# Layr-Labs/rust-kzg-bn254

Measured on AMD Instinct MI355X. Metric: G1-MSM (scalar,point) pairs/s = 2^20 x KZG coeff-form commitments/s, 2^20-point SRS, higher is better.
Workload: dtype int32x9 (29-bit limbs, 64-bit accumulate); 1 GPU; G1 MSM 2^20 scalars (KZG::commit_coeff_form), scalars resident in HBM; step k commits buffer k mod 8 (8 distinct resident scalar sets, 256 MiB); pipeline_depth=2, steps_per_launch=1

## Files before the change

rust-kzg-bn254_amd/csrc/msm_kernels.h:

```cpp
#pragma once
#include <hip/hip_runtime.h>
#include "curve_pair.h"
#include "curve_quad.h"
#include "naf.h"
#include "msm_limits.h"

namespace kzg {

__device__ __forceinline__ void latency_bound_kernel() {
#if !defined(KZG_NO_SETPRIO)
    __builtin_amdgcn_s_setprio(3);
#endif
}

constexpr uint32_t DIGIT_NONE = 0xFFFFFFFFu;

__global__ void __launch_bounds__(256)
k_msm_digits(const uint4* __restrict__ scalars, uint32_t n_total, uint32_t n, int c, int W, uint32_t* __restrict__ digits,
             uint32_t* __restrict__ count = nullptr ) {
    latency_bound_kernel();
    uint32_t j = blockIdx.x * blockDim.x + threadIdx.x;
    if (j >= n_total) return;
    const uint32_t msm = j / n, i = j - msm * n;
    uint4 lo = scalars[2 * (size_t)j], hi = scalars[2 * (size_t)j + 1];
    uint32_t w32[8] = {lo.x, lo.y, lo.z, lo.w, hi.x, hi.y, hi.z, hi.w};
    uint32_t k[8];
    fe_wire_to_canonical_words<FrParams>(k, w32);
    const uint32_t mask = (1u << c) - 1u, half = 1u << (c - 1);
    uint32_t carry = 0;
    for (int w = 0; w < W; ++w) {
        uint32_t raw = (k[0] & mask) + carry;
#pragma unroll
        for (int j = 0; j < 7; ++j) k[j] = (k[j] >> c) | (k[j + 1] << (32 - c));
        k[7] >>= c;
        uint32_t neg = raw > half;
        uint32_t mag = neg ? (1u << c) - raw : raw;
        carry = neg;
        uint32_t v = DIGIT_NONE;
        if (mag != 0) {
            v = (mag - 1) | (neg << 31);
            if (count) atomicAdd(&count[mag - 1], 1u);
        }
        digits[((size_t)msm * W + w) * n + i] = v;
    }
}


template <int T>
__device__ __forceinline__ uint32_t block_excl_scan(uint32_t v, uint32_t* total, uint32_t* lds ) {
    const int t = threadIdx.x;
    lds[t] = v;
    __syncthreads();
    for (int d = 1; d < T; d <<= 1) {
        uint32_t x = (t >= d) ? lds[t - d] : 0u;
        __syncthreads();
        lds[t] += x;
        __syncthreads();
    }
    uint32_t incl = lds[t];
    *total = lds[T - 1];
    __syncthreads();
    return incl - v;
}
__device__ __forceinline__ uint4 scan1_load(const uint32_t* __restrict__ count, uint32_t g, uint32_t hi) {
    if (g + 4 <= hi) return *reinterpret_cast<const uint4*>(count + g);
    uint4 v = make_uint4(0, 0, 0, 0);
    if (g < hi) v.x = count[g];
    if (g + 1 < hi) v.y = count[g + 1];
    if (g + 2 < hi) v.z = count[g + 2];
    return v;
}
template <bool LEAN>
__global__ void __launch_bounds__(SCAN1_THREADS)
k_scan_counts_1wg(uint32_t* __restrict__ count, uint32_t G, uint32_t* __restrict__ offs , uint32_t* __restrict__ cursor ) {
    latency_bound_kernel();
    __shared__ uint32_t wave_total[SCAN1_THREADS / 64];
    const uint32_t t = threadIdx.x, w = t >> 6, lane = t & 63;
    const uint32_t per_wave = (((G + SCAN1_THREADS / 64 - 1) / (SCAN1_THREADS / 64)) + 255u) & ~255u;
    const uint32_t lo = min(G, w * per_wave), hi = min(G, lo + per_wave);
    uint32_t s = 0;
    for (uint32_t g0 = lo; g0 < hi; g0 += 1024) {
        const uint32_t g = g0 + lane * 4;
        const uint4 a = scan1_load(count, g, hi), b = scan1_load(count, g + 256, hi), c = scan1_load(count, g + 512, hi), d = scan1_load(count, g + 768, hi);
        s += a.x + a.y + a.z + a.w + b.x + b.y + b.z + b.w + c.x + c.y + c.z + c.w + d.x + d.y + d.z + d.w;
    }
    for (int d = 32; d >= 1; d >>= 1) s += __shfl_xor(s, d, 64);
    if (lane == 0) wave_total[w] = s;
    __syncthreads();
    uint32_t run = 0, total = 0;
    for (uint32_t q = 0; q < SCAN1_THREADS / 64; ++q) { const uint32_t x = wave_total[q]; if (q < w) run += x; total += x; }
    for (uint32_t g0 = lo; g0 < hi; g0 += 1024) {
        uint4 v[4];
#pragma unroll
        for (int k = 0; k < 4; ++k) v[k] = scan1_load(count, g0 + k * 256 + lane * 4, hi);
#pragma unroll
        for (int k = 0; k < 4; ++k) {
            const uint32_t g = g0 + k * 256 + lane * 4;
            const uint32_t sum4 = v[k].x + v[k].y + v[k].z + v[k].w;
            uint32_t incl = sum4;
            for (int d = 1; d < 64; d <<= 1) { const uint32_t x = __shfl_up(incl, d, 64); if ((int)lane >= d) incl += x; }
            uint4 o;
            o.x = run + incl - sum4; o.y = o.x + v[k].x; o.z = o.y + v[k].y; o.w = o.z + v[k].z;
            if (g + 4 <= hi) {
                *reinterpret_cast<uint4*>(offs + g) = o;
                if (LEAN) { *reinterpret_cast<uint4*>(cursor + g) = o; *reinterpret_cast<uint4*>(count + g) = make_uint4(0, 0, 0, 0); }
            } else {
                if (g < hi) { offs[g] = o.x; if (LEAN) { cursor[g] = o.x; count[g] = 0; } }
                if (g + 1 < hi) { offs[g + 1] = o.y; if (LEAN) { cursor[g + 1] = o.y; count[g + 1] = 0; } }
                if (g + 2 < hi) { offs[g + 2] = o.z; if (LEAN) { cursor[g + 2] = o.z; count[g + 2] = 0; } }
            }
            run += __shfl(incl, 63, 64);
        }
    }
    if (t == 0) offs[G] = total;
}
__global__ void __launch_bounds__(SCAN_THREADS)
k_scan_block_sums(const uint32_t* __restrict__ count, uint32_t G, uint32_t* __restrict__ block_sums) {
    __shared__ uint32_t lds[SCAN_THREADS];
    size_t base = (size_t)blockIdx.x * SCAN_TILE + (size_t)threadIdx.x * SCAN_ITEMS;
    uint32_t s = 0;
#pragma unroll
    for (int j = 0; j < SCAN_ITEMS; ++j) if (base + j < G) s += count[base + j];
    uint32_t total;
    block_excl_scan<SCAN_THREADS>(s, &total, lds);
    if (threadIdx.x == 0) block_sums[blockIdx.x] = total;
}
__global__ void __launch_bounds__(SCAN_THREADS)
k_scan_top(uint32_t* __restrict__ block_sums, uint32_t nb) {
    __shared__ uint32_t lds[SCAN_THREADS];
    size_t base = (size_t)threadIdx.x * SCAN_ITEMS;
    uint32_t v[SCAN_ITEMS], s = 0;
#pragma unroll
    for (int j = 0; j < SCAN_ITEMS; ++j) { v[j] = (base + j < nb) ? block_sums[base + j] : 0u; s += v[j]; }
    uint32_t total;
    uint32_t pre = block_excl_scan<SCAN_THREADS>(s, &total, lds);
#pragma unroll
    for (int j = 0; j < SCAN_ITEMS; ++j) { if (base + j < nb) block_sums[base + j] = pre; pre += v[j]; }
}
__global__ void __launch_bounds__(SCAN_THREADS)
k_scan_final(const uint32_t* __restrict__ count, uint32_t G, const uint32_t* __restrict__ block_sums,
             uint32_t* __restrict__ offs ) {
    __shared__ uint32_t lds[SCAN_THREADS];
    size_t base = (size_t)blockIdx.x * SCAN_TILE + (size_t)threadIdx.x * SCAN_ITEMS;
    uint32_t v[SCAN_ITEMS], s = 0;
#pragma unroll
    for (int j = 0; j < SCAN_ITEMS; ++j) { v[j] = (base + j < G) ? count[base + j] : 0u; s += v[j]; }
    uint32_t total;
    uint32_t pre = block_excl_scan<SCAN_THREADS>(s, &total, lds) + block_sums[blockIdx.x];
#pragma unroll
    for (int j = 0; j < SCAN_ITEMS; ++j) { if (base + j < G) offs[base + j] = pre; pre += v[j]; }
    if (blockIdx.x == gridDim.x - 1 && threadIdx.x == SCAN_THREADS - 1) offs[G] = pre;
}

__global__ void __launch_bounds__(256)
k_sort_hist(const uint32_t* __restrict__ digits, uint32_t set_len, uint32_t tile_len, uint32_t tiles_per_set, uint32_t B,
            uint32_t* __restrict__ count, uint32_t* __restrict__ blockbase) {
    latency_bound_kernel();
    extern __shared__ uint32_t lds_u32[];
    const uint32_t set = blockIdx.x / tiles_per_set, tile = blockIdx.x % tiles_per_set;
    const uint32_t lo = tile * tile_len;
    const uint32_t hi = (set_len - lo < tile_len) ? set_len : lo + tile_len;
    for (uint32_t b = threadIdx.x; b < B; b += blockDim.x) lds_u32[b] = 0;
    __syncthreads();
    const uint32_t* d = digits + (size_t)set * set_len;
    for (uint32_t e = lo + threadIdx.x; e < hi; e += blockDim.x) {
        uint32_t v = d[e];
        if (v != DIGIT_NONE) atomicAdd(&lds_u32[v & 0x7FFFFFFFu], 1u);
    }
    __syncthreads();
    for (uint32_t b = threadIdx.x; b < B; b += blockDim.x) {
        uint32_t h = lds_u32[b];
        uint32_t base = h ? atomicAdd(&count[(size_t)set * B + b], h) : 0u;
        blockbase[(size_t)blockIdx.x * B + b] = base;
    }
}
__global__ void __launch_bounds__(256)
k_sort_scatter(const uint32_t* __restrict__ digits, uint32_t n, uint32_t set_len, uint32_t tile_len, uint32_t tiles_per_set, uint32_t B,
               const uint32_t* __restrict__ offs, const uint32_t* __restrict__ blockbase, uint32_t table_stride,
               uint32_t windows_per_msm, uint32_t* __restrict__ sorted) {
    latency_bound_kernel();
    extern __shared__ uint32_t lds_u32[];
    const uint32_t set = blockIdx.x / tiles_per_set, tile = blockIdx.x % tiles_per_set;
    const uint32_t base_idx = table_stride ? 0u : (set / windows_per_msm) * n;
    const uint32_t lo = tile * tile_len;
    const uint32_t hi = (set_len - lo < tile_len) ? set_len : lo + tile_len;
    for (uint32_t b = threadIdx.x; b < B; b += blockDim.x)
        lds_u32[b] = offs[(size_t)set * B + b] + blockbase[(size_t)blockIdx.x * B + b];
    __syncthreads();
    const uint32_t* d = digits + (size_t)set * set_len;
    for (uint32_t e = lo + threadIdx.x; e < hi; e += blockDim.x) {
        uint32_t v = d[e];
        if (v == DIGIT_NONE) continue;
        uint32_t pos = atomicAdd(&lds_u32[v & 0x7FFFFFFFu], 1u);
        uint32_t idx;
        if (table_stride) { uint32_t w = e / n; idx = w * table_stride + (e - w * n); }
        else idx = base_idx + e;
        sorted[pos] = idx | (v & 0x80000000u);
    }
}

__global__ void __launch_bounds__(256)
k_sort_small_hist(const uint32_t* __restrict__ digits, uint32_t n_entries, uint32_t set_len, uint32_t B, uint32_t* __restrict__ count) {
    latency_bound_kernel();
    const uint32_t e = blockIdx.x * blockDim.x + threadIdx.x;
    if (e >= n_entries) return;
    const uint32_t v = digits[e];
    if (v != DIGIT_NONE) atomicAdd(&count[(size_t)(e / set_len) * B + (v & 0x7FFFFFFFu)], 1u);
}
__global__ void __launch_bounds__(256)
k_sort_small_scatter(const uint32_t* __restrict__ digits, uint32_t n_entries, uint32_t n, uint32_t set_len, uint32_t B,
                     const uint32_t* __restrict__ offs, uint32_t* __restrict__ cursor , uint32_t table_stride,
                     uint32_t windows_per_msm, uint32_t* __restrict__ sorted, int cursor_is_offs = 0) {
    latency_bound_kernel();
    const uint32_t e = blockIdx.x * blockDim.x + threadIdx.x;
    if (e >= n_entries) return;
    const uint32_t v = digits[e];
    if (v == DIGIT_NONE) return;
    const uint32_t set = e / set_len, es = e - set * set_len;
    const size_t gb = (size_t)set * B + (v & 0x7FFFFFFFu);
    const uint32_t pos = (cursor_is_offs ? 0u : offs[gb]) + atomicAdd(&cursor[gb], 1u);
    uint32_t idx;
    if (table_stride) { const uint32_t w = es / n; idx = w * table_stride + (es - w * n); }
    else idx = (set / windows_per_msm) * n + es;
    sorted[pos] = idx | (v & 0x80000000u);
}


template <bool SCATTER>
__global__ void __launch_bounds__(256)
k_sort2_scalars(const uint4* __restrict__ scalars, uint32_t n, int c, int W, uint32_t tile_s, uint32_t Hb, uint32_t* __restrict__ ccount,
                uint32_t* __restrict__ blockbase1, const uint32_t* __restrict__ cstart, uint32_t table_stride, uint32_t* __restrict__ tmp1) {
    latency_bound_kernel();
    extern __shared__ uint32_t lds_u32[];
    const uint32_t lo = blockIdx.x * tile_s;
    const uint32_t hi = (n - lo < tile_s) ? n : lo + tile_s;
    for (uint32_t b = threadIdx.x; b < Hb; b += blockDim.x) lds_u32[b] = SCATTER ? cstart[b] + blockbase1[(size_t)blockIdx.x * Hb + b] : 0u;
    __syncthreads();
    const uint32_t mask = (1u << c) - 1u, half = 1u << (c - 1);
    for (uint32_t i = lo + threadIdx.x; i < hi; i += blockDim.x) {
        const uint4 s_lo = scalars[2 * (size_t)i], s_hi = scalars[2 * (size_t)i + 1];
        uint32_t w32[8] = {s_lo.x, s_lo.y, s_lo.z, s_lo.w, s_hi.x, s_hi.y, s_hi.z, s_hi.w};
        uint32_t k[8];
        fe_wire_to_canonical_words<FrParams>(k, w32);
        uint32_t carry = 0, idx = i;
        for (int w = 0; w < W; ++w, idx += table_stride) {
            const uint32_t raw = (k[0] & mask) + carry;
#pragma unroll
            for (int j = 0; j < 7; ++j) k[j] = (k[j] >> c) | (k[j + 1] << (32 - c));
            k[7] >>= c;
            const uint32_t neg = raw > half;
            const uint32_t mag = neg ? (1u << c) - raw : raw;
            carry = neg;
            if (mag == 0) continue;
            const uint32_t key = mag - 1;
            if (SCATTER) {
                const uint32_t pos = atomicAdd(&lds_u32[key >> SORT2_LO_BITS], 1u);
                tmp1[pos] = (neg << 31) | ((key & (SORT2_LO - 1)) << SORT2_IDX_BITS) | idx;
            } else {
                atomicAdd(&lds_u32[key >> SORT2_LO_BITS], 1u);
            }
        }
    }
    if (SCATTER) return;
    __syncthreads();
    for (uint32_t b = threadIdx.x; b < Hb; b += blockDim.x) {
        const uint32_t h = lds_u32[b];
        blockbase1[(size_t)blockIdx.x * Hb + b] = h ? atomicAdd(&ccount[b], h) : 0u;
    }
}
struct PolyPtrs { const uint4* p[MSM_BATCH_PTRS]; };
template <int ND>
__global__ void __launch_bounds__(256)
k_naf_digits(const uint4* __restrict__ scalars, uint32_t n, int c, uint32_t tile_s, uint32_t Hb, uint32_t* __restrict__ ccount,
             uint32_t* __restrict__ blockbase1, uint4* __restrict__ digs, uint32_t poly_len, PolyPtrs ptrs) {
    latency_bound_kernel();
    extern __shared__ uint32_t lds_u32[];
    uint32_t* hist = lds_u32;
    uint32_t* col = hist + Hb + threadIdx.x;
    uint32_t* stage = hist + Hb + 11 * 256;
    const uint32_t t = threadIdx.x;
    const uint32_t lo = blockIdx.x * tile_s;
    const uint32_t hi = (n - lo < tile_s) ? n : lo + tile_s;
    for (uint32_t b = t; b < Hb; b += 256) hist[b] = 0u;
    col[8 * 256] = 0; col[9 * 256] = 0; col[10 * 256] = 0;
    for (uint32_t base = lo; base < hi; base += 256) {
        __syncthreads();
#pragma unroll
        for (int m = 0; m < ND; ++m) stage[m * 256 + t] = NAF_NO_DIGIT;
        const uint32_t i = base + t;
        if (i < hi) {
            const uint4* sp = scalars + 2 * (size_t)i;
            if (poly_len && ptrs.p[0]) {
                const uint32_t pk = i / poly_len;
                const uint4* base = ptrs.p[0];
#pragma unroll
                for (int q = 1; q < MSM_BATCH_PTRS; ++q) base = pk == (uint32_t)q ? ptrs.p[q] : base;
                sp = base + 2 * (size_t)(i - pk * poly_len);
            }
            const uint4 s_lo = sp[0], s_hi = sp[1];
            uint32_t w32[8] = {s_lo.x, s_lo.y, s_lo.z, s_lo.w, s_hi.x, s_hi.y, s_hi.z, s_hi.w};
            uint32_t k[8];
            fe_wire_to_canonical_words<FrParams>(k, w32);
#pragma unroll
            for (int j = 0; j < 8; ++j) col[j * 256] = k[j];
            uint32_t m = 0;
            const uint32_t group = poly_len ? (i / poly_len) << (c - 1) : 0u;
            naf_for_digits_lds(col, 256, c + 1, [&](uint32_t pos, uint32_t key, uint32_t neg) {
                const uint32_t g = group | (c - 1 > 6 ? naf_bucket(key, c - 1) : key);
                atomicAdd(&hist[g >> SORT2_LO_BITS], 1u);
                if (m < (uint32_t)ND) stage[m * 256 + t] = (neg << 31) | (pos << 16) | g;
                ++m;
            });
        }
        __syncthreads();
#pragma unroll
        for (int r = 0; r < ND / 4; ++r) {
            const uint32_t idx = t + 256 * r, sc = idx / (ND / 4), q = idx % (ND / 4);
            if (base + sc < hi)
                digs[(size_t)(base + sc) * (ND / 4) + q] = make_uint4(stage[(4 * q) * 256 + sc], stage[(4 * q + 1) * 256 + sc],
                                                                    stage[(4 * q + 2) * 256 + sc], stage[(4 * q + 3) * 256 + sc]);
        }
    }
    __syncthreads();
    for (uint32_t b = t; b < Hb; b += 256) {
        const uint32_t h = hist[b];
        blockbase1[(size_t)blockIdx.x * Hb + b] = h ? atomicAdd(&ccount[b], h) : 0u;
    }
}
static_assert(SORT2_MAX_BINS <= 512 && SORT2_LO_BITS == 7, "LDS entry layout of k_sort2_scatter1_lds");
template <class F>
__device__ __forceinline__ void sort2_for_digits(uint32_t k[8], int c, int W, F&& f) {
    const uint32_t mask = (1u << c) - 1u, half = 1u << (c - 1);
    uint32_t carry = 0;
    for (int w = 0; w < W; ++w) {
        const uint32_t raw = (k[0] & mask) + carry;
#pragma unroll
        for (int j = 0; j < 7; ++j) k[j] = (k[j] >> c) | (k[j + 1] << (32 - c));
        k[7] >>= c;
        const uint32_t neg = raw > half;
        const uint32_t mag = neg ? (1u << c) - raw : raw;
        carry = neg;
        if (mag != 0) f((uint32_t)w, mag - 1, neg);
    }
}
template <bool NAF = false, int ND = NAF_DIGITS>
__global__ void __launch_bounds__(SORT2_P1_THREADS)
k_sort2_scatter1_lds(const uint4* __restrict__ scalars, uint32_t n, int c, int W, uint32_t tile_s, uint32_t Hb, const uint32_t* __restrict__ blockbase1,
                     const uint32_t* __restrict__ cstart, uint32_t table_stride, uint32_t* __restrict__ tmp1, uint8_t* __restrict__ tmpk = nullptr,
                     uint32_t poly_len = 0) {
    latency_bound_kernel();
    extern __shared__ uint32_t lds_u32[];
    uint32_t* gpos = lds_u32;
    uint32_t* hist = gpos + Hb;
    uint32_t* lstart = hist + Hb;
    uint32_t* buf = lstart + Hb;
    uint16_t* bufk = reinterpret_cast<uint16_t*>(buf + (size_t)SORT2_P1_THREADS * W);
    const uint32_t t = threadIdx.x, lane = t & 63;
    const uint32_t lo = blockIdx.x * tile_s;
    const uint32_t hi = (n - lo < tile_s) ? n : lo + tile_s;
    for (uint32_t b = t; b < Hb; b += SORT2_P1_THREADS) gpos[b] = cstart[b] + blockbase1[(size_t)blockIdx.x * Hb + b];
    const uint32_t per_lane = (Hb + 63) / 64;
    for (uint32_t base = lo; base < hi; base += SORT2_P1_THREADS) {
        __syncthreads();
        for (uint32_t b = t; b < Hb; b += SORT2_P1_THREADS) hist[b] = 0;
        __syncthreads();
        const uint32_t i = base + t;
        const bool have = i < hi;
        uint32_t kk[8] = {0, 0, 0, 0, 0, 0, 0, 0};
        uint32_t dg[NAF ? ND : 1];
        if (NAF) {
#pragma unroll
            for (int m = 0; m < (NAF ? ND : 1); ++m) dg[m] = NAF_NO_DIGIT;
            if (have) {
                const uint4* src = reinterpret_cast<const uint4*>(scalars) + (size_t)i * (ND / 4);
#pragma unroll
                for (int q = 0; q < (NAF ? ND / 4 : 0); ++q) {
                    const uint4 v = src[q];
                    dg[4 * q] = v.x; dg[4 * q + 1] = v.y; dg[4 * q + 2] = v.z; dg[4 * q + 3] = v.w;
                }
                bool live = true;
#pragma unroll
                for (int m = 0; m < (NAF ? ND : 0); ++m) {
                    live = live && dg[m] != NAF_NO_DIGIT;
                    if (!live) dg[m] = NAF_NO_DIGIT;
                    else atomicAdd(&hist[(dg[m] & 0xFFFFu) >> SORT2_LO_BITS], 1u);
                }
            }
        } else
        if (have) {
            const uint4 s_lo = scalars[2 * (size_t)i], s_hi = scalars[2 * (size_t)i + 1];
            const uint32_t w32[8] = {s_lo.x, s_lo.y, s_lo.z, s_lo.w, s_hi.x, s_hi.y, s_hi.z, s_hi.w};
            fe_wire_to_canonical_words<FrParams>(kk, w32);
            uint32_t k[8];
#pragma unroll
            for (int j = 0; j < 8; ++j) k[j] = kk[j];
            sort2_for_digits(k, c, W, [&](uint32_t, uint32_t key, uint32_t) { atomicAdd(&hist[key >> SORT2_LO_BITS], 1u); });
        }
        __syncthreads();
        if (t < 64) {
            uint32_t sum = 0;
            for (uint32_t q = 0; q < per_lane; ++q) { const uint32_t b = lane * per_lane + q; if (b < Hb) sum += hist[b]; }
            uint32_t incl = sum;
            for (int d = 1; d < 64; d <<= 1) { const uint32_t x = __shfl_up(incl, d, 64); if ((int)lane >= d) incl += x; }
            uint32_t run = incl - sum;
            for (uint32_t q = 0; q < per_lane; ++q) {
                const uint32_t b = lane * per_lane + q;
                if (b < Hb) { lstart[b] = run; run += hist[b]; }
            }
        }
        __syncthreads();
        const uint32_t cn = lstart[Hb - 1] + hist[Hb - 1];
        __syncthreads();
        for (uint32_t b = t; b < Hb; b += SORT2_P1_THREADS) hist[b] = 0;
        __syncthreads();
        if (have) {
            if (NAF) {
#pragma unroll
                for (int m = 0; m < (NAF ? ND : 0); ++m) {
                    if (dg[m] == NAF_NO_DIGIT) continue;
                    const uint32_t key = dg[m] & 0xFFFFu;
                    const uint32_t bin = key >> SORT2_LO_BITS;
                    const uint32_t slot = lstart[bin] + atomicAdd(&hist[bin], 1u);
                    buf[slot] = (dg[m] & 0x80000000u) | (((dg[m] >> 16) & 255u) << 9) | t;
                    bufk[slot] = (uint16_t)key;
                }
            } else {
                sort2_for_digits(kk, c, W, [&](uint32_t w, uint32_t key, uint32_t neg) {
                    const uint32_t bin = key >> SORT2_LO_BITS;
                    const uint32_t slot = lstart[bin] + atomicAdd(&hist[bin], 1u);
                    buf[slot] = (bin << 22) | ((key & (SORT2_LO - 1)) << 15) | (neg << 14) | (w << 9) | t;
                });
            }
        }
        __syncthreads();
        if (NAF) {
            for (uint32_t q = t; q < cn; q += SORT2_P1_THREADS) {
                const uint32_t x = buf[q], key = bufk[q], bin = key >> SORT2_LO_BITS;
                const uint32_t sidx = base + (x & 511u);
                const uint32_t idx = ((x >> 9) & 255u) * table_stride + (poly_len ? sidx % poly_len : sidx);
                const uint32_t dst = gpos[bin] + (q - lstart[bin]);
                tmp1[dst] = (x & 0x80000000u) | idx;
                tmpk[dst] = (uint8_t)(key & (SORT2_LO - 1));
            }
        } else
        for (uint32_t q = t; q < cn; q += SORT2_P1_THREADS) {
            const uint32_t x = buf[q], bin = x >> 22;
            const uint32_t idx = ((x >> 9) & 31u) * table_stride + base + (x & 511u);
            tmp1[gpos[bin] + (q - lstart[bin])] = ((x >> 14) & 1u) << 31 | ((x >> 15) & (SORT2_LO - 1)) << SORT2_IDX_BITS | idx;
        }
        __syncthreads();
        for (uint32_t b = t; b < Hb; b += SORT2_P1_THREADS) gpos[b] += hist[b];
    }
}
__global__ void __launch_bounds__(512)
k_sort2_scan(const uint32_t* __restrict__ ccount, uint32_t Hb, uint32_t* __restrict__ cstart, uint32_t* __restrict__ tstart,
             uint32_t* __restrict__ tile_bin, uint32_t* __restrict__ count, uint32_t* __restrict__ cap_out) {
    latency_bound_kernel();
    __shared__ uint32_t a[512], b[512];
    __shared__ uint32_t total;
    const uint32_t t = threadIdx.x;
    uint32_t c = t < Hb ? ccount[t] : 0u;
    if (t == 0) total = 0;
    __syncthreads();
    if (c) atomicAdd(&total, c);
    __syncthreads();
    const uint32_t cap_dyn = total / Hb + total / Hb / 4 + 2048u;
    const uint32_t cap = cap_dyn < SORT2_BIN_CAP ? cap_dyn : SORT2_BIN_CAP;
    if (t == 0) *cap_out = cap;
    uint32_t k = c > cap ? (c + SORT2_CHUNK - 1) / SORT2_CHUNK : 0u;
    a[t] = c; b[t] = k;
    __syncthreads();
    for (uint32_t d = 1; d < 512; d <<= 1) {
        uint32_t x = t >= d ? a[t - d] : 0u, y = t >= d ? b[t - d] : 0u;
        __syncthreads();
        a[t] += x; b[t] += y;
        __syncthreads();
    }
    if (t < Hb) {
        cstart[t] = a[t] - c; tstart[t] = b[t] - k;
        for (uint32_t q = b[t] - k; q < b[t]; ++q) tile_bin[q] = t;
        if (k) for (uint32_t q = 0; q < SORT2_LO; ++q) count[(size_t)t * SORT2_LO + q] = 0u;
    }
    if (t == Hb - 1) { cstart[Hb] = a[t]; tstart[Hb] = b[t]; }
}
template <bool NAF>
__device__ __forceinline__ uint32_t sort2_low_key(const uint32_t* __restrict__ tmp1, const uint8_t* __restrict__ tmpk, uint32_t e) {
    return NAF ? (uint32_t)tmpk[e] : (tmp1[e] >> SORT2_IDX_BITS) & (SORT2_LO - 1);
}
template <bool NAF = false>
__global__ void __launch_bounds__(256)
k_sort2_hist2(const uint32_t* __restrict__ tmp1, const uint32_t* __restrict__ cstart, const uint32_t* __restrict__ tstart,
              const uint32_t* __restrict__ tile_bin, uint32_t Hb, uint32_t* __restrict__ count, uint32_t* __restrict__ blockbase2,
              const uint8_t* __restrict__ tmpk = nullptr) {
    latency_bound_kernel();
    __shared__ uint32_t hist[SORT2_LO];
    const uint32_t tile = blockIdx.x;
    if (tile >= tstart[Hb]) return;
    const uint32_t h = tile_bin[tile];
    const uint32_t lo = cstart[h] + (tile - tstart[h]) * SORT2_CHUNK;
    const uint32_t hi = (cstart[h + 1] - lo < SORT2_CHUNK) ? cstart[h + 1] : lo + SORT2_CHUNK;
    if (threadIdx.x < SORT2_LO) hist[threadIdx.x] = 0;
    __syncthreads();
    for (uint32_t e = lo + threadIdx.x; e < hi; e += blockDim.x) atomicAdd(&hist[sort2_low_key<NAF>(tmp1, tmpk, e)], 1u);
    __syncthreads();
    if (threadIdx.x < SORT2_LO) {
        uint32_t c = hist[threadIdx.x];
        blockbase2[(size_t)tile * SORT2_LO + threadIdx.x] = c ? atomicAdd(&count[(size_t)h * SORT2_LO + threadIdx.x], c) : 0u;
    }
}
template <bool NAF = false>
__global__ void __launch_bounds__(256)
k_sort2_scatter2(const uint32_t* __restrict__ tmp1, const uint32_t* __restrict__ cstart, const uint32_t* __restrict__ tstart,
                 const uint32_t* __restrict__ tile_bin, uint32_t Hb, const uint32_t* __restrict__ offs,
                 const uint32_t* __restrict__ blockbase2, uint32_t* __restrict__ sorted, const uint8_t* __restrict__ tmpk = nullptr) {
    latency_bound_kernel();
    __shared__ uint32_t cur[SORT2_LO];
    const uint32_t tile = blockIdx.x;
    if (tile >= tstart[Hb]) return;
    const uint32_t h = tile_bin[tile];
    const uint32_t lo = cstart[h] + (tile - tstart[h]) * SORT2_CHUNK;
    const uint32_t hi = (cstart[h + 1] - lo < SORT2_CHUNK) ? cstart[h + 1] : lo + SORT2_CHUNK;
    if (threadIdx.x < SORT2_LO)
        cur[threadIdx.x] = offs[(size_t)h * SORT2_LO + threadIdx.x] + blockbase2[(size_t)tile * SORT2_LO + threadIdx.x];
    __syncthreads();
    for (uint32_t e = lo + threadIdx.x; e < hi; e += blockDim.x) {
        uint32_t v = tmp1[e];
        uint32_t pos = atomicAdd(&cur[sort2_low_key<NAF>(tmp1, tmpk, e)], 1u);
        sorted[pos] = NAF ? v : v & (0x80000000u | SORT2_IDX_MASK);
    }
}

template <bool NAF = false>
__global__ void __launch_bounds__(SORT2_BIN_THREADS)
k_sort2_bin(const uint32_t* __restrict__ tmp1, const uint32_t* __restrict__ cstart, uint32_t Hb, const uint32_t* __restrict__ count,
            uint32_t* __restrict__ offs, uint32_t* __restrict__ sorted, const uint32_t* __restrict__ cap_ptr, const uint8_t* __restrict__ tmpk = nullptr) {
    latency_bound_kernel();
    __shared__ uint32_t hist[SORT2_LO], gpos[SORT2_LO], lstart[SORT2_LO], buf[SORT2_BIN_CHUNK];
    __shared__ uint8_t bufk[NAF ? SORT2_BIN_CHUNK : 4];
    const uint32_t h = blockIdx.x, t = threadIdx.x;
    const uint32_t lo = cstart[h], hi = cstart[h + 1];
    const bool large = hi - lo > *cap_ptr;
    if (t < SORT2_LO) hist[t] = large ? count[(size_t)h * SORT2_LO + t] : 0u;
    __syncthreads();
    if (!large) {
        uint32_t e = lo + t;
        for (; e + 3 * SORT2_BIN_THREADS < hi; e += 4 * SORT2_BIN_THREADS) {
            const uint32_t k0 = sort2_low_key<NAF>(tmp1, tmpk, e), k1 = sort2_low_key<NAF>(tmp1, tmpk, e + SORT2_BIN_THREADS),
                           k2 = sort2_low_key<NAF>(tmp1, tmpk, e + 2 * SORT2_BIN_THREADS), k3 = sort2_low_key<NAF>(tmp1, tmpk, e + 3 * SORT2_BIN_THREADS);
            atomicAdd(&hist[k0], 1u);
            atomicAdd(&hist[k1], 1u);
            atomicAdd(&hist[k2], 1u);
            atomicAdd(&hist[k3], 1u);
        }
        for (; e < hi; e += SORT2_BIN_THREADS) atomicAdd(&hist[sort2_low_key<NAF>(tmp1, tmpk, e)], 1u);
        __syncthreads();
    }
    static_assert(SORT2_LO == 128, "two counters per lane of one wave");
    if (t < 64) {
        const uint32_t c0 = hist[2 * t], c1 = hist[2 * t + 1];
        uint32_t incl = c0 + c1;
        for (int d = 1; d < 64; d <<= 1) { const uint32_t x = __shfl_up(incl, d, 64); if ((int)t >= d) incl += x; }
        const uint32_t start = lo + incl - (c0 + c1);
        gpos[2 * t] = start; gpos[2 * t + 1] = start + c0;
        offs[(size_t)h * SORT2_LO + 2 * t] = start;
        offs[(size_t)h * SORT2_LO + 2 * t + 1] = start + c0;
    }
    if (h == Hb - 1 && t == 0) offs[(size_t)Hb * SORT2_LO] = cstart[Hb];
    if (large) return;
    for (uint32_t base = lo; base < hi; base += SORT2_BIN_CHUNK) {
        const uint32_t cn = hi - base < SORT2_BIN_CHUNK ? hi - base : SORT2_BIN_CHUNK;
        __syncthreads();
        if (t < SORT2_LO) hist[t] = 0;
        __syncthreads();
        uint32_t v[SORT2_BIN_PER], r[SORT2_BIN_PER], kq[SORT2_BIN_PER];
#pragma unroll
        for (int j = 0; j < SORT2_BIN_PER; ++j) {
            const uint32_t i = j * SORT2_BIN_THREADS + t;
            v[j] = i < cn ? tmp1[base + i] : 0u;
            kq[j] = NAF ? (i < cn ? (uint32_t)tmpk[base + i] : 0u) : (v[j] >> SORT2_IDX_BITS) & (SORT2_LO - 1);
        }
#pragma unroll
        for (int j = 0; j < SORT2_BIN_PER; ++j)
            if (j * SORT2_BIN_THREADS + t < cn) r[j] = atomicAdd(&hist[kq[j]], 1u);
        __syncthreads();
        if (t < 64) {
            const uint32_t c0 = hist[2 * t], c1 = hist[2 * t + 1];
            uint32_t incl = c0 + c1;
            for (int d = 1; d < 64; d <<= 1) { const uint32_t x = __shfl_up(incl, d, 64); if ((int)t >= d) incl += x; }
            lstart[2 * t] = incl - (c0 + c1); lstart[2 * t + 1] = incl - c1;
        }
        __syncthreads();
#pragma unroll
        for (int j = 0; j < SORT2_BIN_PER; ++j)
            if (j * SORT2_BIN_THREADS + t < cn) {
                const uint32_t slot = lstart[kq[j]] + r[j];
                buf[slot] = v[j];
                if (NAF) bufk[slot] = (uint8_t)kq[j];
            }
        __syncthreads();
        for (uint32_t i = t; i < cn; i += SORT2_BIN_THREADS) {
            const uint32_t x = buf[i], k = NAF ? (uint32_t)bufk[i] : (x >> SORT2_IDX_BITS) & (SORT2_LO - 1);
            sorted[gpos[k] + (i - lstart[k])] = NAF ? x : x & (0x80000000u | SORT2_IDX_MASK);
        }
        __syncthreads();
        if (t < SORT2_LO) gpos[t] += hist[t];
    }
}

#ifndef KZG_RUN_SERIAL
#define KZG_RUN_SERIAL 8
#endif
constexpr uint32_t RUN_SERIAL = KZG_RUN_SERIAL;
constexpr uint32_t NP_SERIAL = 10;

__device__ __forceinline__ uint32_t acc_seg_len(uint32_t E, uint32_t nl) { return (E + nl - 1) / nl; }

#ifdef KZG_ACC_NOGATHER
#define KZG_ACC_IDX(v) ((v) & 0xFFu)
#else
#define KZG_ACC_IDX(v) ((v) & 0x7FFFFFFFu)
#endif
__device__ __forceinline__ size_t acc_point_index(uint32_t ix, uint32_t idx_log, uint32_t stride_adj) {
    return (size_t)ix + (size_t)(ix >> idx_log) * stride_adj;
}
#ifndef KZG_ACC_WAVES
#define KZG_ACC_WAVES 3
#endif
#ifdef KZG_TEST_HOOKS
__device__ unsigned long long g_acc_replays;
#endif
__device__ __noinline__ Xyzz acc_replay(const uint4* __restrict__ points, const uint32_t* __restrict__ sorted, uint32_t lo, uint32_t hi, uint32_t idx_log, uint32_t stride_adj) {
    Xyzz r;
    xyzz_set_inf(r);
#pragma unroll 1
    for (uint32_t e = lo; e < hi; ++e) {
        const uint32_t v = sorted[e];
        Affine p;
        if (!affine_load(p, points + 4 * acc_point_index(KZG_ACC_IDX(v), idx_log, stride_adj))) continue;
        xyzz_madd<true>(r, p, v >> 31);
    }
#ifdef KZG_TEST_HOOKS
    atomicAdd(&g_acc_replays, 1ull);
#endif
    return r;
}
template <bool IDENTITY_BASES>
__global__ void __launch_bounds__(256) __attribute__((amdgpu_waves_per_eu(KZG_ACC_WAVES, KZG_ACC_WAVES)))
k_msm_accumulate(const uint4* __restrict__ points, const uint32_t* __restrict__ sorted, const uint32_t* __restrict__ offs, uint32_t G,
                 int32_t* __restrict__ head, size_t head_stride, int32_t* __restrict__ cont, size_t cont_stride,
                 uint32_t idx_log, uint32_t stride_adj) {
    const uint32_t nl = gridDim.x * blockDim.x;
    const uint32_t t = blockIdx.x * blockDim.x + threadIdx.x;
    const uint32_t lane = threadIdx.x & 63;
#ifdef KZG_ACC_STAMPS
    unsigned long long* stamps = reinterpret_cast<unsigned long long*>(cont + cont_stride * 36) + 8 * (size_t)(t >> 6);
    const unsigned long long stamp0 = __builtin_amdgcn_s_memrealtime();
    unsigned long long flush_ticks = 0, flush_events = 0, stamp_loop = 0;
#endif
    const uint32_t E = offs[G];
    const uint32_t L = acc_seg_len(E, nl);
    const unsigned long long b64 = (unsigned long long)t * L;
    const uint32_t begin = b64 < E ? (uint32_t)b64 : E;
    const uint32_t end = (b64 + L < E) ? (uint32_t)(b64 + L) : E;
    const bool active = begin < end;
    uint32_t g = 0, next = 0, g0 = 0xFFFFFFFFu;
    bool is_cont = false, long_run = false;
    if (active) {
        uint32_t lo = 0, hi = G;
#ifdef KZG_ACC_BINARY_SEARCH
        while (hi - lo > 1) {
            const uint32_t mid = (lo + hi) >> 1;
            if (offs[mid] <= begin) lo = mid; else hi = mid;
        }
#else
        while (hi - lo > 1) {
            const uint32_t s = (hi - lo + 15) >> 4;
            uint32_t cnt = 0;
#pragma unroll
            for (uint32_t j = 1; j < 16; ++j) {
                const uint32_t p = lo + j * s;
                const uint32_t v = p < hi ? offs[p] : 0xFFFFFFFFu;
                cnt += v <= begin ? 1u : 0u;
            }
            const uint32_t nlo = lo + cnt * s, nhi = lo + (cnt + 1) * s;
            if (cnt < 15 && nhi < hi) hi = nhi;
            lo = nlo;
        }
#endif
        g = lo;
        const uint32_t o0 = offs[g];
        next = offs[g + 1];
        is_cont = o0 < begin;
        if (is_cont) { long_run = ((next - 1) / L - o0 / L) > RUN_SERIAL; g0 = g; }
    }
    __shared__ int32_t park[4 * NL * 256];
    const uint32_t tl = threadIdx.x;
    bool parked = false, parked_cont = false;
    uint32_t park_g = 0;
    bool cont_in_regs = false;
    Xyzz acc;
    xyzz_set_inf(acc);
    uint32_t next2 = 0;
    if (active) next2 = offs[g + 2 <= G ? g + 2 : G];
    auto flush = [&](bool more) {
        if (__builtin_expect(!acc.inf && fe_is_zero_mod(acc.zz), 0)) {
            const uint32_t o0 = offs[g], o1 = offs[g + 1];
            acc = acc_replay(points, sorted, o0 > begin ? o0 : begin, o1 < end ? o1 : end, idx_log, stride_adj);
        }
        KZG_REQUIRE(!acc.inf || (fe_is_literal_zero(acc.x) && fe_is_literal_zero(acc.y) && fe_is_literal_zero(acc.zz) && fe_is_literal_zero(acc.zzz)),
                    KZG_SITE_IS_ZERO_MOD, "k_msm_accumulate: inf without zero limbs", acc.zz);
        const bool as_cont = is_cont && g == g0;
        if (more && !parked) {
            const Fq* c4[4] = {&acc.x, &acc.y, &acc.zz, &acc.zzz};
#pragma unroll
            for (int q = 0; q < 4; ++q)
#pragma unroll
                for (int j = 0; j < NL; ++j) park[(q * NL + j) * 256 + tl] = c4[q]->l[j];
            parked = true; parked_cont = as_cont; park_g = g;
        } else if (!as_cont) {
            xyzz_store_zeroed(head, head_stride, g, acc);
        } else if (!long_run || more) {
            xyzz_store_zeroed(cont, cont_stride, t, acc);
        } else {
            cont_in_regs = true;
        }
    };
#ifdef KZG_ACC_STAMPS
    stamp_loop = __builtin_amdgcn_s_memrealtime();
#endif
    if (active) {
        const uint32_t last = end - 1;
        uint32_t v = sorted[begin];
        uint32_t v1 = sorted[begin + 1 < end ? begin + 1 : last];
        typedef uint32_t u32x4 __attribute__((ext_vector_type(4)));
        const u32x4* const pts = reinterpret_cast<const u32x4*>(points);
        const u32x4* src = pts + 4 * acc_point_index(KZG_ACC_IDX(v), idx_log, stride_adj);
        u32x4 q0 = src[0], q1 = src[1], q2 = src[2], q3 = src[3];
        for (uint32_t e = begin; e < end; ++e) {
#ifdef KZG_ACC_STAMPS
            const bool any_cross = __any(e == next);
            unsigned long long f0 = 0;
            if (any_cross) f0 = __builtin_amdgcn_s_memrealtime();
#endif
            if (__builtin_expect(e == next, 0)) {
                flush(true);
                xyzz_set_inf(acc);
                ++g; next = next2;
                while (next == e) { ++g; next = offs[g + 1]; }
                next2 = offs[g + 2 <= G ? g + 2 : G];
            }
#ifdef KZG_ACC_STAMPS
            if (any_cross) { flush_ticks += __builtin_amdgcn_s_memrealtime() - f0; flush_events += 1; }
#endif
            const uint32_t neg = v >> 31;
            asm("" : "+v"(q0), "+v"(q1), "+v"(q2), "+v"(q3));
            uint32_t wx[8] = {q0.x, q0.y, q0.z, q0.w, q1.x, q1.y, q1.z, q1.w};
            uint32_t wy[8] = {q2.x, q2.y, q2.z, q2.w, q3.x, q3.y, q3.z, q3.w};
            const uint32_t any = q0.x | q0.y | q0.z | q0.w | q1.x | q1.y | q1.z | q1.w | q2.x | q2.y | q2.z | q2.w | q3.x | q3.y | q3.z | q3.w;
            Affine p;
            fe_unpack(p.x, wx);
            fe_unpack(p.y, wy);
            v = v1;
            src = pts + 4 * acc_point_index(KZG_ACC_IDX(v), idx_log, stride_adj);
            q0 = src[0]; q1 = src[1]; q2 = src[2]; q3 = src[3];
            v1 = sorted[e + 2 < end ? e + 2 : last];
            if (IDENTITY_BASES && any == 0) continue;
            xyzz_madd<true, false>(acc, p, neg);
        }
        flush(false);
    }
    const bool in_scan = active && is_cont && long_run;
    Xyzz c;
    xyzz_set_inf(c);
    if (cont_in_regs) c = acc;
    if (parked) {
        Xyzz v;
        Fq* c4[4] = {&v.x, &v.y, &v.zz, &v.zzz};
#pragma unroll
        for (int q = 0; q < 4; ++q)
#pragma unroll
            for (int j = 0; j < NL; ++j) c4[q]->l[j] = park[(q * NL + j) * 256 + tl];
        v.inf = fe_is_literal_zero(v.zz);
        if (!parked_cont) xyzz_store(head, head_stride, park_g, v);
        else if (!long_run) xyzz_store(cont, cont_stride, t, v);
        else c = v;
    }
#ifdef KZG_ACC_STAMPS
    if (lane == 0) {
        unsigned int hwid, xcc;
        asm volatile("s_getreg_b32 %0, hwreg(HW_REG_HW_ID)" : "=s"(hwid));
        asm volatile("s_getreg_b32 %0, hwreg(HW_REG_XCC_ID)" : "=s"(xcc));
        stamps[0] = stamp0; stamps[1] = __builtin_amdgcn_s_memrealtime(); stamps[2] = hwid; stamps[3] = xcc;
        stamps[4] = flush_ticks; stamps[5] = flush_events; stamps[6] = stamp_loop;
    }
#endif
    if (!__any(in_scan)) return;
    const uint32_t key = in_scan ? g0 : 0xFFFFFFFFu;
#pragma unroll 1
    for (int d = 1; d < 64; d <<= 1) {
        const uint32_t kd = __shfl_down(key, d, 64);
        const bool join = in_scan && (lane + d < 64) && kd == key;
        if (!__any(join)) continue;
        Xyzz u;
        xyzz_shfl_down(u, c, d);
        if (join) {
            Xyzz r;
            xyzz_add<true>(r, c, u);
            c = r;
        }
    }
    const uint32_t kprev = __shfl_up(key, 1, 64);
    if (in_scan && (lane == 0 || kprev != key)) xyzz_store(cont, cont_stride, t, c);
}

__device__ __forceinline__ size_t bucket_pos(uint32_t g, uint32_t m, uint32_t n_chunks) {
    return (size_t)(g % m) * n_chunks + (g / m);
}
struct BucketSpan {
    uint32_t g, t1, np;
    bool long_run;
};
__device__ __forceinline__ BucketSpan bucket_span(const uint32_t* __restrict__ offs, uint32_t g, uint32_t L) {
    BucketSpan s;
    s.g = g;
    const uint32_t o0 = offs[g], o1 = offs[g + 1];
    s.t1 = 0; s.np = 0; s.long_run = false;
    if (o1 == o0) return s;
    s.t1 = o0 / L;
    const uint32_t t2 = (o1 - 1) / L, r = t2 - s.t1;
    s.long_run = r > RUN_SERIAL;
    s.np = 1 + (s.long_run ? 1 + (t2 / 64 - (s.t1 + 1) / 64) : r);
    return s;
}
__device__ __forceinline__ uint32_t bucket_cont_lane(const BucketSpan& s, uint32_t k) {
    const uint32_t first = s.t1 + 1;
    return !s.long_run ? s.t1 + k : (k == 1 ? first : (first / 64 + (k - 1)) * 64);
}
__device__ __forceinline__ void bucket_partial(Xyzz& v, const BucketSpan& s, uint32_t k, const int32_t* __restrict__ head, size_t head_stride,
                                               const int32_t* __restrict__ cont, size_t cont_stride) {
    if (k == 0) { xyzz_load(v, head, head_stride, s.g); return; }
    xyzz_load(v, cont, cont_stride, bucket_cont_lane(s, k));
}
__device__ __forceinline__ void bucket_sum_wave(Xyzz& acc, const BucketSpan& s, uint32_t lane, const int32_t* __restrict__ head, size_t head_stride,
                                                const int32_t* __restrict__ cont, size_t cont_stride) {
    xyzz_set_inf(acc);
    const bool heavy = s.np > NP_SERIAL;
    if (!heavy) {
#pragma unroll 1
        for (uint32_t k = 0; k < s.np; ++k) {
            Xyzz v, r;
            bucket_partial(v, s, k, head, head_stride, cont, cont_stride);
            xyzz_add<true>(r, acc, v);
            acc = r;
        }
    }
    unsigned long long todo = __ballot(heavy);
    while (todo) {
        const int src = __ffsll((long long)todo) - 1;
        todo &= todo - 1;
        BucketSpan h;
        h.g = __shfl(s.g, src, 64);
        h.t1 = __shfl(s.t1, src, 64);
        h.np = __shfl(s.np, src, 64);
        h.long_run = __shfl((int)s.long_run, src, 64) != 0;
        Xyzz part;
        xyzz_set_inf(part);
#pragma unroll 1
        for (uint32_t k = lane; k < h.np; k += 64) {
            Xyzz v, r;
            bucket_partial(v, h, k, head, head_stride, cont, cont_stride);
            xyzz_add<true>(r, part, v);
            part = r;
        }
#pragma unroll 1
        for (int d = 32; d >= 1; d >>= 1) {
            Xyzz u, r;
            xyzz_shfl_down(u, part, d);
            xyzz_add<true>(r, part, u);
            part = r;
        }
        Xyzz tot;
        const Fq* sp[4] = {&part.x, &part.y, &part.zz, &part.zzz};
        Fq* tp[4] = {&tot.x, &tot.y, &tot.zz, &tot.zzz};
#pragma unroll
        for (int q = 0; q < 4; ++q)
#pragma unroll
            for (int j = 0; j < NL; ++j) tp[q]->l[j] = __shfl(sp[q]->l[j], 0, 64);
        tot.inf = __shfl((int)part.inf, 0, 64) != 0;
        if ((int)lane == src) acc = tot;
    }
}

__global__ void __launch_bounds__(256) __attribute__((amdgpu_waves_per_eu(3, 3)))
k_msm_bucket_fin(const uint32_t* __restrict__ offs, uint32_t G, uint32_t nl, uint32_t m, uint32_t n_chunks,
                 const int32_t* __restrict__ head, size_t head_stride, const int32_t* __restrict__ cont, size_t cont_stride,
                 int32_t* __restrict__ bucket, size_t bucket_stride) {
    latency_bound_kernel();
    const uint32_t g = blockIdx.x * blockDim.x + threadIdx.x, lane = threadIdx.x & 63;
    const uint32_t L = acc_seg_len(offs[G], nl);
    BucketSpan s;
    s.g = g; s.t1 = 0; s.np = 0; s.long_run = false;
    if (g < G && L) s = bucket_span(offs, g, L);
    Xyzz acc;
    bucket_sum_wave(acc, s, lane, head, head_stride, cont, cont_stride);
    if (g < G) xyzz_store(bucket, bucket_stride, m ? bucket_pos(g, m, n_chunks) : (size_t)g, acc);
}

__global__ void __launch_bounds__(256)
// ... 533 lines not shown
```

Before: 972.5 million pairs/s.

## Streamline sort2 scatter and bin kernels: fewer barriers and counting passes

After: 973.3 million pairs/s, median of 4. About the same (+0.1%).

```diff
diff --git a/rust-kzg-bn254_amd/csrc/msm_kernels.h b/rust-kzg-bn254_amd/csrc/msm_kernels.h
--- a/rust-kzg-bn254_amd/csrc/msm_kernels.h
+++ b/rust-kzg-bn254_amd/csrc/msm_kernels.h
@@ -303,13 +303,15 @@
             fe_wire_to_canonical_words<FrParams>(k, w32);
 #pragma unroll
             for (int j = 0; j < 8; ++j) col[j * 256] = k[j];
-            uint32_t m = 0;
+            uint32_t* slot = stage + t;
+            uint32_t* const slot_end = slot + ND * 256;
             const uint32_t group = poly_len ? (i / poly_len) << (c - 1) : 0u;
+            const uint32_t rot = c - 1 > 6 ? (uint32_t)(c - 7) : 0u;
             naf_for_digits_lds(col, 256, c + 1, [&](uint32_t pos, uint32_t key, uint32_t neg) {
-                const uint32_t g = group | (c - 1 > 6 ? naf_bucket(key, c - 1) : key);
+                const uint32_t g = group | ((key & 63u) << rot) | (key >> 6);
                 atomicAdd(&hist[g >> SORT2_LO_BITS], 1u);
-                if (m < (uint32_t)ND) stage[m * 256 + t] = (neg << 31) | (pos << 16) | g;
-                ++m;
+                if (slot < slot_end) *slot = (neg << 31) | (pos << 16) | g;
+                slot += 256;
             });
         }
         __syncthreads();
@@ -350,24 +352,24 @@
                      uint32_t poly_len = 0) {
     latency_bound_kernel();
     extern __shared__ uint32_t lds_u32[];
+    __shared__ uint32_t chunk_entries;
     uint32_t* gpos = lds_u32;
-    uint32_t* hist = gpos + Hb;
-    uint32_t* lstart = hist + Hb;
-    uint32_t* buf = lstart + Hb;
+    uint32_t* gold = gpos + Hb;
+    uint32_t* lrel = gold + Hb;
+    uint32_t* buf = lrel + Hb;
     uint16_t* bufk = reinterpret_cast<uint16_t*>(buf + (size_t)SORT2_P1_THREADS * W);
     const uint32_t t = threadIdx.x, lane = t & 63;
     const uint32_t lo = blockIdx.x * tile_s;
     const uint32_t hi = (n - lo < tile_s) ? n : lo + tile_s;
-    for (uint32_t b = t; b < Hb; b += SORT2_P1_THREADS) gpos[b] = cstart[b] + blockbase1[(size_t)blockIdx.x * Hb + b];
+    for (uint32_t b = t; b < Hb; b += SORT2_P1_THREADS) gpos[b] = gold[b] = cstart[b] + blockbase1[(size_t)blockIdx.x * Hb + b];
     const uint32_t per_lane = (Hb + 63) / 64;
+    __syncthreads();
     for (uint32_t base = lo; base < hi; base += SORT2_P1_THREADS) {
-        __syncthreads();
-        for (uint32_t b = t; b < Hb; b += SORT2_P1_THREADS) hist[b] = 0;
-        __syncthreads();
         const uint32_t i = base + t;
         const bool have = i < hi;
         uint32_t kk[8] = {0, 0, 0, 0, 0, 0, 0, 0};
-        uint32_t dg[NAF ? ND : 1];
+        uint32_t dg[NAF ? ND : 1], rk[NAF ? ND : 1];
+        int nd = 0;
         if (NAF) {
 #pragma unroll
             for (int m = 0; m < (NAF ? ND : 1); ++m) dg[m] = NAF_NO_DIGIT;
@@ -378,13 +380,14 @@
                     const uint4 v = src[q];
                     dg[4 * q] = v.x; dg[4 * q + 1] = v.y; dg[4 * q + 2] = v.z; dg[4 * q + 3] = v.w;
                 }
-                bool live = true;
-#pragma unroll
-                for (int m = 0; m < (NAF ? ND : 0); ++m) {
-                    live = live && dg[m] != NAF_NO_DIGIT;
-                    if (!live) dg[m] = NAF_NO_DIGIT;
-                    else atomicAdd(&hist[(dg[m] & 0xFFFFu) >> SORT2_LO_BITS], 1u);
-                }
+            }
+#pragma unroll
+            for (int m = 0; m < (NAF ? ND : 0); ++m) {
+                if (nd != m) continue;
+                const bool live = dg[m] != NAF_NO_DIGIT;
+                if (__ballot(live) == 0) continue;
+                nd = m + 1;
+                if (live) rk[m] = atomicAdd(&gpos[(dg[m] & 0xFFFFu) >> SORT2_LO_BITS], 1u);
             }
         } else
         if (have) {
@@ -394,62 +397,59 @@
             uint32_t k[8];
 #pragma unroll
             for (int j = 0; j < 8; ++j) k[j] = kk[j];
-            sort2_for_digits(k, c, W, [&](uint32_t, uint32_t key, uint32_t) { atomicAdd(&hist[key >> SORT2_LO_BITS], 1u); });
+            sort2_for_digits(k, c, W, [&](uint32_t, uint32_t key, uint32_t) { atomicAdd(&gpos[key >> SORT2_LO_BITS], 1u); });
         }
         __syncthreads();
         if (t < 64) {
             uint32_t sum = 0;
-            for (uint32_t q = 0; q < per_lane; ++q) { const uint32_t b = lane * per_lane + q; if (b < Hb) sum += hist[b]; }
+            for (uint32_t q = 0; q < per_lane; ++q) { const uint32_t b = lane * per_lane + q; if (b < Hb) sum += gpos[b] - gold[b]; }
             uint32_t incl = sum;
             for (int d = 1; d < 64; d <<= 1) { const uint32_t x = __shfl_up(incl, d, 64); if ((int)lane >= d) incl += x; }
             uint32_t run = incl - sum;
             for (uint32_t q = 0; q < per_lane; ++q) {
                 const uint32_t b = lane * per_lane + q;
-                if (b < Hb) { lstart[b] = run; run += hist[b]; }
-            }
-        }
-        __syncthreads();
-        const uint32_t cn = lstart[Hb - 1] + hist[Hb - 1];
-        __syncthreads();
-        for (uint32_t b = t; b < Hb; b += SORT2_P1_THREADS) hist[b] = 0;
-        __syncthreads();
-        if (have) {
-            if (NAF) {
-#pragma unroll
-                for (int m = 0; m < (NAF ? ND : 0); ++m) {
-                    if (dg[m] == NAF_NO_DIGIT) continue;
-                    const uint32_t key = dg[m] & 0xFFFFu;
-                    const uint32_t bin = key >> SORT2_LO_BITS;
-                    const uint32_t slot = lstart[bin] + atomicAdd(&hist[bin], 1u);
-                    buf[slot] = (dg[m] & 0x80000000u) | (((dg[m] >> 16) & 255u) << 9) | t;
-                    bufk[slot] = (uint16_t)key;
+                if (b < Hb) {
+                    const uint32_t g = gpos[b], o = gold[b];
+                    lrel[b] = run - o; run += g - o;
+                    if (NAF) gold[b] = g;
                 }
-            } else {
-                sort2_for_digits(kk, c, W, [&](uint32_t w, uint32_t key, uint32_t neg) {
-                    const uint32_t bin = key >> SORT2_LO_BITS;
-                    const uint32_t slot = lstart[bin] + atomicAdd(&hist[bin], 1u);
-                    buf[slot] = (bin << 22) | ((key & (SORT2_LO - 1)) << 15) | (neg << 14) | (w << 9) | t;
-                });
-            }
+            }
+            if (lane == 63) chunk_entries = incl;
         }
         __syncthreads();
         if (NAF) {
+#pragma unroll
+            for (int m = 0; m < (NAF ? ND : 0); ++m) {
+                if (m >= nd || dg[m] == NAF_NO_DIGIT) continue;
+                const uint32_t key = dg[m] & 0xFFFFu;
+                const uint32_t slot = lrel[key >> SORT2_LO_BITS] + rk[m];
+                buf[slot] = (dg[m] & 0x80000000u) | (((dg[m] >> 16) & 255u) << 9) | t;
+                bufk[slot] = (uint16_t)key;
+            }
+        } else if (have) {
+            sort2_for_digits(kk, c, W, [&](uint32_t w, uint32_t key, uint32_t neg) {
+                const uint32_t bin = key >> SORT2_LO_BITS;
+                const uint32_t slot = lrel[bin] + atomicAdd(&gold[bin], 1u);
+                buf[slot] = (bin << 22) | ((key & (SORT2_LO - 1)) << 15) | (neg << 14) | (w << 9) | t;
+            });
+        }
+        __syncthreads();
+        const uint32_t cn = chunk_entries;
+        if (NAF) {
             for (uint32_t q = t; q < cn; q += SORT2_P1_THREADS) {
-                const uint32_t x = buf[q], key = bufk[q], bin = key >> SORT2_LO_BITS;
+                const uint32_t x = buf[q], key = bufk[q];
                 const uint32_t sidx = base + (x & 511u);
                 const uint32_t idx = ((x >> 9) & 255u) * table_stride + (poly_len ? sidx % poly_len : sidx);
-                const uint32_t dst = gpos[bin] + (q - lstart[bin]);
+                const uint32_t dst = q - lrel[key >> SORT2_LO_BITS];
                 tmp1[dst] = (x & 0x80000000u) | idx;
                 tmpk[dst] = (uint8_t)(key & (SORT2_LO - 1));
             }
         } else
         for (uint32_t q = t; q < cn; q += SORT2_P1_THREADS) {
-            const uint32_t x = buf[q], bin = x >> 22;
+            const uint32_t x = buf[q];
             const uint32_t idx = ((x >> 9) & 31u) * table_stride + base + (x & 511u);
-            tmp1[gpos[bin] + (q - lstart[bin])] = ((x >> 14) & 1u) << 31 | ((x >> 15) & (SORT2_LO - 1)) << SORT2_IDX_BITS | idx;
-        }
-        __syncthreads();
-        for (uint32_t b = t; b < Hb; b += SORT2_P1_THREADS) gpos[b] += hist[b];
+            tmp1[q - lrel[x >> 22]] = ((x >> 14) & 1u) << 31 | ((x >> 15) & (SORT2_LO - 1)) << SORT2_IDX_BITS | idx;
+        }
     }
 }
 __global__ void __launch_bounds__(512)
@@ -531,79 +531,107 @@
 }
 
 template <bool NAF = false>
-__global__ void __launch_bounds__(SORT2_BIN_THREADS)
+__global__ void __launch_bounds__(SORT2_BIN_THREADS, 8)
 k_sort2_bin(const uint32_t* __restrict__ tmp1, const uint32_t* __restrict__ cstart, uint32_t Hb, const uint32_t* __restrict__ count,
             uint32_t* __restrict__ offs, uint32_t* __restrict__ sorted, const uint32_t* __restrict__ cap_ptr, const uint8_t* __restrict__ tmpk = nullptr) {
     latency_bound_kernel();
-    __shared__ uint32_t hist[SORT2_LO], gpos[SORT2_LO], lstart[SORT2_LO], buf[SORT2_BIN_CHUNK];
+    __shared__ uint32_t gpos[SORT2_LO], gold[SORT2_LO], lrel[SORT2_LO], buf[SORT2_BIN_CHUNK];
     __shared__ uint8_t bufk[NAF ? SORT2_BIN_CHUNK : 4];
     const uint32_t h = blockIdx.x, t = threadIdx.x;
     const uint32_t lo = cstart[h], hi = cstart[h + 1];
     const bool large = hi - lo > *cap_ptr;
-    if (t < SORT2_LO) hist[t] = large ? count[(size_t)h * SORT2_LO + t] : 0u;
-    __syncthreads();
-    if (!large) {
-        uint32_t e = lo + t;
-        for (; e + 3 * SORT2_BIN_THREADS < hi; e += 4 * SORT2_BIN_THREADS) {
-            const uint32_t k0 = sort2_low_key<NAF>(tmp1, tmpk, e), k1 = sort2_low_key<NAF>(tmp1, tmpk, e + SORT2_BIN_THREADS),
-                           k2 = sort2_low_key<NAF>(tmp1, tmpk, e + 2 * SORT2_BIN_THREADS), k3 = sort2_low_key<NAF>(tmp1, tmpk, e + 3 * SORT2_BIN_THREADS);
-            atomicAdd(&hist[k0], 1u);
-            atomicAdd(&hist[k1], 1u);
-            atomicAdd(&hist[k2], 1u);
-            atomicAdd(&hist[k3], 1u);
-        }
-        for (; e < hi; e += SORT2_BIN_THREADS) atomicAdd(&hist[sort2_low_key<NAF>(tmp1, tmpk, e)], 1u);
-        __syncthreads();
-    }
-    static_assert(SORT2_LO == 128, "two counters per lane of one wave");
-    if (t < 64) {
-        const uint32_t c0 = hist[2 * t], c1 = hist[2 * t + 1];
-        uint32_t incl = c0 + c1;
-        for (int d = 1; d < 64; d <<= 1) { const uint32_t x = __shfl_up(incl, d, 64); if ((int)t >= d) incl += x; }
-        const uint32_t start = lo + incl - (c0 + c1);
-        gpos[2 * t] = start; gpos[2 * t + 1] = start + c0;
-        offs[(size_t)h * SORT2_LO + 2 * t] = start;
-        offs[(size_t)h * SORT2_LO + 2 * t + 1] = start + c0;
-    }
-    if (h == Hb - 1 && t == 0) offs[(size_t)Hb * SORT2_LO] = cstart[Hb];
-    if (large) return;
-    for (uint32_t base = lo; base < hi; base += SORT2_BIN_CHUNK) {
-        const uint32_t cn = hi - base < SORT2_BIN_CHUNK ? hi - base : SORT2_BIN_CHUNK;
-        __syncthreads();
-        if (t < SORT2_LO) hist[t] = 0;
-        __syncthreads();
-        uint32_t v[SORT2_BIN_PER], r[SORT2_BIN_PER], kq[SORT2_BIN_PER];
+    const bool one = !large && hi - lo <= SORT2_BIN_CHUNK;
+    uint32_t v[SORT2_BIN_PER], r[SORT2_BIN_PER], kq[SORT2_BIN_PER];
+    auto load_chunk = [&](uint32_t base, uint32_t cn) {
 #pragma unroll
         for (int j = 0; j < SORT2_BIN_PER; ++j) {
             const uint32_t i = j * SORT2_BIN_THREADS + t;
             v[j] = i < cn ? tmp1[base + i] : 0u;
             kq[j] = NAF ? (i < cn ? (uint32_t)tmpk[base + i] : 0u) : (v[j] >> SORT2_IDX_BITS) & (SORT2_LO - 1);
         }
+    };
+    if (t < SORT2_LO) gpos[t] = large ? count[(size_t)h * SORT2_LO + t] : 0u;
+    __syncthreads();
+    if (one) {
+        load_chunk(lo, hi - lo);
 #pragma unroll
         for (int j = 0; j < SORT2_BIN_PER; ++j)
-            if (j * SORT2_BIN_THREADS + t < cn) r[j] = atomicAdd(&hist[kq[j]], 1u);
+            if (j * SORT2_BIN_THREADS + t < hi - lo) r[j] = atomicAdd(&gpos[kq[j]], 1u);
         __syncthreads();
-        if (t < 64) {
-            const uint32_t c0 = hist[2 * t], c1 = hist[2 * t + 1];
-            uint32_t incl = c0 + c1;
-            for (int d = 1; d < 64; d <<= 1) { const uint32_t x = __shfl_up(incl, d, 64); if ((int)t >= d) incl += x; }
-            lstart[2 * t] = incl - (c0 + c1); lstart[2 * t + 1] = incl - c1;
+    } else if (!large) {
+        if (NAF) {
+            const uint32_t a = (lo + 15u) & ~15u, b = a + ((hi - a) & ~15u);
+            if (lo + t < a) atomicAdd(&gpos[tmpk[lo + t]], 1u);
+            for (uint32_t e = a + 16u * t; e < b; e += 16u * SORT2_BIN_THREADS) {
+                const uint4 q = *reinterpret_cast<const uint4*>(tmpk + e);
+                const uint32_t w4[4] = {q.x, q.y, q.z, q.w};
+#pragma unroll
+                for (int j = 0; j < 4; ++j) {
+                    atomicAdd(&gpos[w4[j] & 255u], 1u);
+                    atomicAdd(&gpos[(w4[j] >> 8) & 255u], 1u);
+                    atomicAdd(&gpos[(w4[j] >> 16) & 255u], 1u);
+                    atomicAdd(&gpos[w4[j] >> 24], 1u);
+                }
+            }
+            if (b + t < hi) atomicAdd(&gpos[tmpk[b + t]], 1u);
+        } else {
+            uint32_t e = lo + t;
+            for (; e + 3 * SORT2_BIN_THREADS < hi; e += 4 * SORT2_BIN_THREADS) {
+                const uint32_t k0 = sort2_low_key<NAF>(tmp1, tmpk, e), k1 = sort2_low_key<NAF>(tmp1, tmpk, e + SORT2_BIN_THREADS),
+                               k2 = sort2_low_key<NAF>(tmp1, tmpk, e + 2 * SORT2_BIN_THREADS), k3 = sort2_low_key<NAF>(tmp1, tmpk, e + 3 * SORT2_BIN_THREADS);
+                atomicAdd(&gpos[k0], 1u);
+                atomicAdd(&gpos[k1], 1u);
+                atomicAdd(&gpos[k2], 1u);
+                atomicAdd(&gpos[k3], 1u);
+            }
+            for (; e < hi; e += SORT2_BIN_THREADS) atomicAdd(&gpos[sort2_low_key<NAF>(tmp1, tmpk, e)], 1u);
         }
         __syncthreads();
+    }
+    static_assert(SORT2_LO == 128, "two counters per lane of one wave");
+    if (t < 64) {
+        const uint32_t c0 = gpos[2 * t], c1 = gpos[2 * t + 1];
+        uint32_t incl = c0 + c1;
+        for (int d = 1; d < 64; d <<= 1) { const uint32_t x = __shfl_up(incl, d, 64); if ((int)t >= d) incl += x; }
+        const uint32_t start = lo + incl - (c0 + c1);
+        gpos[2 * t] = gold[2 * t] = start; gpos[2 * t + 1] = gold[2 * t + 1] = start + c0;
+        lrel[2 * t] = start - lo; lrel[2 * t + 1] = start + c0 - lo;
+        offs[(size_t)h * SORT2_LO + 2 * t] = start;
+        offs[(size_t)h * SORT2_LO + 2 * t + 1] = start + c0;
+    }
+    if (h == Hb - 1 && t == 0) offs[(size_t)Hb * SORT2_LO] = cstart[Hb];
+    if (large) return;
+    __syncthreads();
+    for (uint32_t base = lo; base < hi; base += SORT2_BIN_CHUNK) {
+        const uint32_t cn = hi - base < SORT2_BIN_CHUNK ? hi - base : SORT2_BIN_CHUNK;
+        if (!one) {
+            load_chunk(base, cn);
+#pragma unroll
+            for (int j = 0; j < SORT2_BIN_PER; ++j)
+                if (j * SORT2_BIN_THREADS + t < cn) r[j] = atomicAdd(&gpos[kq[j]], 1u);
+            __syncthreads();
+            if (t < 64) {
+                const uint32_t g0 = gpos[2 * t], g1 = gpos[2 * t + 1], o0 = gold[2 * t], o1 = gold[2 * t + 1];
+                const uint32_t c0 = g0 - o0, c1 = g1 - o1;
+                uint32_t incl = c0 + c1;
+                for (int d = 1; d < 64; d <<= 1) { const uint32_t x = __shfl_up(incl, d, 64); if ((int)t >= d) incl += x; }
+                lrel[2 * t] = incl - (c0 + c1) - o0; lrel[2 * t + 1] = incl - c1 - o1;
+                gold[2 * t] = g0; gold[2 * t + 1] = g1;
+            }
+            __syncthreads();
+        }
 #pragma unroll
         for (int j = 0; j < SORT2_BIN_PER; ++j)
             if (j * SORT2_BIN_THREADS + t < cn) {
-                const uint32_t slot = lstart[kq[j]] + r[j];
+                const uint32_t slot = lrel[kq[j]] + r[j];
                 buf[slot] = v[j];
                 if (NAF) bufk[slot] = (uint8_t)kq[j];
             }
         __syncthreads();
         for (uint32_t i = t; i < cn; i += SORT2_BIN_THREADS) {
             const uint32_t x = buf[i], k = NAF ? (uint32_t)bufk[i] : (x >> SORT2_IDX_BITS) & (SORT2_LO - 1);
-            sorted[gpos[k] + (i - lstart[k])] = NAF ? x : x & (0x80000000u | SORT2_IDX_MASK);
-        }
-        __syncthreads();
-        if (t < SORT2_LO) gpos[t] += hist[t];
+            sorted[one ? lo + i : i - lrel[k]] = NAF ? x : x & (0x80000000u | SORT2_IDX_MASK);
+        }
     }
 }
 
```
